# HKUST-Aerial-Robotics/A-LOAM

Hardware: AMD Instinct MI355X
Metric: HDL-64 scans/sec (whole node) (higher is better)
Workload: dtype f32 features / f64 solve

## Files before the change

a-loam_amd/binding.py:

```python
from __future__ import annotations

import ctypes as C
import os
import re
import subprocess

import numpy as np

_HERE = os.path.dirname(os.path.abspath(__file__))
_ROOT = os.path.dirname(_HERE)
LIB_PATH = os.path.join(_HERE, "lib", "libaloam_mi355x.so")
HEADER_PATH = os.path.join(_ROOT, "include", "aloam_mi355x.h")

CLOUD_FULL, CLOUD_SHARP, CLOUD_LESS_SHARP, CLOUD_FLAT, CLOUD_LESS_FLAT, CLOUD_CORNER_LAST, CLOUD_SURF_LAST = range(7)
E_ARG, E_SCAN_LINES, E_EMPTY, E_CAPACITY, E_HIP, E_STATE = -1, -2, -3, -4, -5, -6
MAP_REGISTERED, MAP_CORNER_STACK, MAP_SURF_STACK, MAP_SURROUND, MAP_FULL = 2, 3, 4, 5, 6
EXPORT_MAP, EXPORT_MAX_IDS = 16, 12
STAGE_REGISTRATION, STAGE_ODOMETRY, STAGE_MAPPING, STAGE_ALL = 1, 2, 4, 7
SEQ_RECORD_MAGIC, SEQ_RECORD_VERSION = 0x51534C41, 1
SEQ_PART_ODOMETRY, SEQ_PART_MAP = 1, 2
MAP_INFO_KEYS = ("cenW", "cenH", "cenD", "frame_count", "from_map_corner", "from_map_surf", "corner_stack", "surf_stack",
                 "corner_num0", "corner_num1", "surf_num0", "surf_num1", "lm_iterations0", "lm_iterations1", "termination0", "compactions")


# ... 316 lines not shown
        L.aloam_atlas_attach.argtypes = [vp, vp]
        L.aloam_atlas_info.argtypes = [vp, vp]
        L.aloam_places_enable.argtypes = [vp, C.c_int, C.c_float, C.c_float]
        L.aloam_places_add.argtypes = [vp, vp, C.c_int]
        L.aloam_places_match.argtypes = [vp, vp, C.c_int, vp, C.c_int, vp]
        L.aloam_places_export.argtypes = [vp, C.c_int, C.c_int, vp]
        L.aloam_places_load.argtypes = [vp, vp, C.c_int]
        L.aloam_places_clear.argtypes = [vp]
        L.aloam_places_info.argtypes = [vp, vp]
        L.aloam_save_sequences.argtypes = [vp, vp, C.c_int, vp, C.c_longlong, vp]
        L.aloam_load_sequences.argtypes = [vp, vp, C.c_int, vp, vp]
        L.aloam_get_ring_ranges.argtypes = [vp, C.c_int, vp, vp]
        L.aloam_get_curvature.argtypes = [vp, C.c_int, vp, C.c_int]
        L.aloam_get_labels.argtypes = [vp, C.c_int, vp, C.c_int]
        L.aloam_get_last_cloud_order.argtypes = [vp, C.c_int, vp]
        L.aloam_get_correspondences.argtypes = [vp, C.c_int, vp, C.c_int, ip, vp, vp, C.c_int, ip, vp]
        L.aloam_mapping_enable.argtypes = [vp, C.c_float, C.c_float, C.c_int]
        L.aloam_mapping_step.argtypes = [vp]
        L.aloam_mapping_set_pool_limit.argtypes = [vp, C.c_int]
        L.aloam_get_map_pool_info.argtypes = [vp, vp]
        L.aloam_set_map.argtypes = [vp, C.c_int, C.c_int, vp, vp, C.c_int, vp]
        L.aloam_set_map_frame.argtypes = [vp, C.c_int, vp, vp, vp, C.c_int]
        L.aloam_set_full_cloud.argtypes = [vp, C.c_int, vp, C.c_int]
        L.aloam_get_map_pose.argtypes = [vp, C.c_int, vp, vp, vp, vp]
        L.aloam_get_map_info.argtypes = [vp, C.c_int, vp]
        L.aloam_map_cube_counts.argtypes = [vp, C.c_int, C.c_int, vp]
        L.aloam_get_map_cube.argtypes = [vp, C.c_int, C.c_int, C.c_int, vp, C.c_int]
        L.aloam_get_map_cloud.argtypes = [vp, C.c_int, C.c_int, vp, C.c_int]
        L.aloam_export_poses.argtypes = [vp, vp]
        L.aloam_export_clouds.argtypes = [vp, vp, C.c_int, vp, C.c_longlong, vp]
# ... 662 lines not shown
    def pose(self, seq=0):
        qw, tw, ql, tl = np.zeros(4), np.zeros(3), np.zeros(4), np.zeros(3)
        self._check(lib().aloam_get_pose(self.h, seq, _p(qw), _p(tw), _p(ql), _p(tl)))
        return {"q_w": qw, "t_w": tw, "q_lc": ql, "t_lc": tl}

    def odom_stats(self, seq=0):
        st = AloamOdomStats()
        self._check(lib().aloam_get_odom_stats(self.h, seq, C.byref(st)))
        return {k: list(getattr(st, k)) for k, _ in AloamOdomStats._fields_}

    def last_cloud_order(self, seq=0):
        v = np.zeros(2, np.int32)
        self._check(lib().aloam_get_last_cloud_order(self.h, seq, _p(v)))
        return int(v[0]), int(v[1])

    def correspondences(self, seq=0):
        cap_e, cap_p = self.n_scans * 12, self.n_scans * 24
        e = np.zeros((cap_e, 9), np.float32); p = np.zeros((cap_p, 12), np.float32)
        eq = np.zeros(cap_e, np.int32); pq = np.zeros(cap_p, np.int32)
        ne, npl = C.c_int(0), C.c_int(0)
        self._check(lib().aloam_get_correspondences(self.h, seq, _p(e), cap_e, C.byref(ne), _p(eq), _p(p), cap_p, C.byref(npl), _p(pq)))
        return e[:ne.value].copy(), p[:npl.value].copy(), eq[:ne.value].copy(), pq[:npl.value].copy()

    def mapping_enable(self, line_res=0.4, plane_res=0.8, pool_points=262144, pool_limit=None):
        if pool_limit is not None:
            self._check(lib().aloam_mapping_set_pool_limit(self.h, int(pool_limit)))
        self._check(lib().aloam_mapping_enable(self.h, float(line_res), float(plane_res), int(pool_points)))

    def map_pool_info(self):
        v = np.zeros(4, np.int32)
# ... 101 lines not shown
```

a-loam_amd/csrc/aloam_capi.hip:

```cpp
#include <algorithm>
#include <cstdio>
#include <cstdlib>
#include <cstring>

#include "capi_internal.hpp"
#include "information_device.hpp"

namespace aloam {

hipEvent_t prof_event(aloam_ctx* c) {
  if (!c->prof_free.empty()) { hipEvent_t e = c->prof_free.back(); c->prof_free.pop_back(); return e; }
  Event e;
  (void)hipEventCreate(&e.h);
  c->prof_events.push_back(std::move(e));
  return c->prof_events.back();
}

int stage_ints(aloam_ctx* c, const int* src, int n, int* dst) {
  int* slot = nullptr;
  int ns = 0;
  if (const int rc = c->nin.acquire(c, &slot, &ns)) return rc;
  std::memcpy(slot, src, sizeof(int) * n);
  return c->nin.queue(c, ns, slot, sizeof(int) * n, dst, c->stream);
}
// ... 77 lines not shown
  int ndev = 0;
  if (hipGetDeviceCount(&ndev) != hipSuccess || ndev <= 0) { c->err = "no HIP device available (this library has no CPU fallback)"; return ALOAM_E_HIP; }
  if (cfg->device < 0 || cfg->device >= ndev) { c->err = "device ordinal out of range"; return ALOAM_E_ARG; }
  DeviceScope device_scope(c);
  HIP_TRY(c, hipStreamCreateWithFlags(&c->stream.h, hipStreamNonBlocking));
  HIP_TRY(c, hipStreamCreateWithFlags(&c->copy_stream.h, hipStreamNonBlocking));
  for (int k = 0; k < 2; ++k) {
    HIP_TRY(c, hipEventCreateWithFlags(&c->in_copied[k].h, hipEventDisableTiming));
    HIP_TRY(c, hipEventCreateWithFlags(&c->in_consumed[k].h, hipEventDisableTiming));
  }
  c->B = cfg->batch; c->max_points = cfg->max_points; c->R = cfg->n_scans;
  c->seq.assign(c->B, SeqHost{});
  c->cap = cfg->max_points + (((cfg->max_points / 32 + 15) & ~15) + 16);
  { const char* e = std::getenv("ALOAM_GRAPH_MAX_BATCH"); c->use_graph = c->B <= (e ? std::atoi(e) : 0); }
  { const char* e = std::getenv("ALOAM_GRID_OVERLAP"); c->grid_overlap = !(e && e[0] == '0') && !c->use_graph && !c->debug_sync; }
  c->NB = (c->cap + kBlockPts - 1) / kBlockPts;
  c->npad = cfg->max_ring_points <= 2059 ? 2048 : 4096;
  const size_t B = c->B, cap = c->cap, R = c->R, NB = c->NB;
  int rc = 0;
  if (const char* what = c->nin.create(sizeof(int) * B)) { c->err = std::string("input counts, ") + what; return ALOAM_E_HIP; }
  const bool reg = stages & ALOAM_STAGE_REGISTRATION, odo = stages & ALOAM_STAGE_ODOMETRY, map = stages & ALOAM_STAGE_MAPPING;
  c->grid_H[0] = R > 64 ? 8192 : 4096;
  c->grid_H[1] = c->max_points > 160000 ? 32768 : 16384;
  if ((rc = dmalloc(c, c->d_nin, B))) return rc;
  if ((rc = dmalloc(c, c->d_meta, B))) return rc;
  if ((rc = dmalloc(c, c->d_state, B))) return rc;
  if ((rc = dmalloc(c, c->d_cloud, B * cap))) return rc;
  if ((rc = dmalloc(c, c->d_exp_cnt, B * ALOAM_EXPORT_MAX_IDS))) return rc;
  if ((rc = dmalloc(c, c->d_exp_chunk, B * ALOAM_EXPORT_MAX_IDS + 1))) return rc;
  if ((rc = dmalloc(c, c->d_exp_off, B * ALOAM_EXPORT_MAX_IDS + 1))) return rc;
// ... 28 lines not shown
      if ((rc = dmalloc(c, c->d_grid_sorted3c[p][k], B * per))) return rc;
      if ((rc = dmalloc(c, c->d_grid_start3c[p][k], B * (c->grid_H[k] + 1)))) return rc;
      if ((rc = dmalloc(c, c->d_grid_flags[p][k], B * 4))) return rc;
      if ((rc = dmalloc(c, c->d_grid_walk[p][k], B * 2 * (R + 8)))) return rc;
    }
    if (c->grid_overlap) {
      HIP_TRY(c, hipStreamCreateWithFlags(&c->grid_stream.h, hipStreamNonBlocking));
      HIP_TRY(c, hipEventCreateWithFlags(&c->grid_fork.h, hipEventDisableTiming));
      HIP_TRY(c, hipEventCreateWithFlags(&c->grids_done.h, hipEventDisableTiming));
    }
    if ((rc = dmalloc(c, c->d_edges, B * R * kSharpPerRing))) return rc;
    if ((rc = dmalloc(c, c->d_planes, B * R * kFlatPerRing))) return rc;
    if ((rc = dmalloc(c, c->d_sel_sharp, B * R * kSharpPerRing))) return rc;
    if ((rc = dmalloc(c, c->d_sel_flat, B * R * kFlatPerRing))) return rc;
    if ((rc = prepare_build_grids(c->grid_H[1]))) { c->err = "k_build_grids: dynamic LDS size rejected"; return ALOAM_E_HIP; }
  }
  std::vector<OdomState> init(B);
  std::memset(init.data(), 0, sizeof(OdomState) * B);
  for (size_t b = 0; b < B; ++b) { init[b].para_q[3] = 1.0; init[b].q_w[3] = 1.0; }
  HIP_TRY(c, hipMemcpyAsync(c->d_state.get(), init.data(), sizeof(OdomState) * B, hipMemcpyHostToDevice, c->stream));
  HIP_TRY(c, hipStreamSynchronize(c->stream));
  return ALOAM_OK;
}

void aloam_destroy(aloam_ctx* c) {
  DeviceScope device_scope(c);
  if (!c) return;
  if (c->stream) (void)hipStreamSynchronize(c->stream);
  if (c->copy_stream) (void)hipStreamSynchronize(c->copy_stream);
  if (c->grid_stream) (void)hipStreamSynchronize(c->grid_stream);
// ... 184 lines not shown
```

a-loam_amd/csrc/aloam_device.hpp:

```cpp
#pragma once
#include <hip/hip_runtime.h>
#include <stdint.h>
#include "aloam_atan.hpp"

namespace aloam {

constexpr int kFrontSlots = 128 + 8;
constexpr int kBlockPts = 1024;
constexpr int kMaxRings = 128;
constexpr int kSectors = 6;
constexpr int kSharpPerSector = 2;
constexpr int kLessSharpPerSector = 20;
constexpr int kFlatPerSector = 4;
constexpr int kSharpPerRing = kSectors * kSharpPerSector;
constexpr int kLessSharpPerRing = kSectors * kLessSharpPerSector;
constexpr int kFlatPerRing = kSectors * kFlatPerSector;
constexpr int kNnTile = 1024;

enum ErrBits { kErrEmpty = 1, kErrRingCap = 2, kErrPointCap = 4, kErrInternal = 8 };

struct alignas(16) SeqMeta {
  int n_in;
  int first_kept, last_kept;
  int half_idx;
// ... 75 lines not shown
  int* grid_start3[2][2];
  int* grid_start2[2][2];
  float4* grid_sorted3c[2][2];
  int* grid_start3c[2][2];
  int* grid_flags[2][2];
  int* grid_walk[2][2];
  int grid_H_corner, grid_H_surf;
  float4* sel_sharp;
  float4* sel_flat;
  EdgeRec* edges;
  PlaneRec* planes;
  int outer;
  int last_outer;
  int lm_max_iterations;
  int distortion;
};

template <typename T>
__device__ __forceinline__ T* row_of(T* const (&buf)[2], int k, int b, long long per) { return (k ? buf[1] : buf[0]) + b * per; }
__device__ __forceinline__ const float4* corner_last(const OdomArgs& a, int b, int parity) { return row_of(a.less_sharp, parity ^ 1, b, (long long)a.R * kLessSharpPerRing); }
__device__ __forceinline__ const float4* surf_last(const OdomArgs& a, int b, int parity) { return row_of(a.less_flat, parity ^ 1, b, (long long)a.cap); }

struct GridView {
  int H;
  float4 *sorted3, *sorted2, *sorted3c;
  int *start3, *start2, *start3c, *flags, *walk;
};
template <typename T>
__device__ __forceinline__ T* grid_ptr(T* const (&buf)[2][2], int set, int which) {
  return set ? (which ? buf[1][1] : buf[1][0]) : (which ? buf[0][1] : buf[0][0]);
// ... 259 lines not shown
```

a-loam_amd/csrc/capi_internal.hpp:

```cpp
#pragma once
#include <hip/hip_runtime.h>

#include <cstdio>
#include <memory>
#include <functional>
#include <string>
#include <utility>
#include <vector>

#include "../../include/aloam_mi355x.h"
#include "aloam_device.hpp"
#include "atlas_kernels.hpp"
#include "checkpoint_kernels.hpp"
#include "export_kernels.hpp"
#include "graphapply_kernels.hpp"
#include "graphmap_kernels.hpp"
#include "graphmarginal_kernels.hpp"
#include "graphrecord_kernels.hpp"
#include "loopreg_kernels.hpp"
#include "loopsearch_kernels.hpp"
#include "mapping_kernels.hpp"
#include "odometry_kernels.hpp"
#include "places_kernels.hpp"
#include "posegraph_kernels.hpp"
// ... 191 lines not shown
  bool dense_valid = true;
  DevBuf<int> d_ringstart;
  DevBuf<float4> d_cloud; DevBuf<float> d_curv; DevBuf<int8_t> d_label;
  DevBuf<unsigned long long> d_lookback; unsigned reg_epoch = 0;
  DevBuf<int> d_ring_ticket;
  bool debug_arrays = false;
  DevBuf<float4> d_sharp, d_flat;
  DevBuf<float4> d_less_sharp[2], d_less_flat[2];
  DevBuf<OdomState> d_state;
  DevBuf<float4> d_grid_sorted3[2][2], d_grid_sorted2[2][2];
  DevBuf<int> d_grid_start3[2][2], d_grid_start2[2][2];
  DevBuf<float4> d_grid_sorted3c[2][2];
  DevBuf<int> d_grid_start3c[2][2];
  DevBuf<int> d_grid_flags[2][2], d_grid_walk[2][2];
  int grid_H[2] = {4096, 16384};
  bool grid_overlap = false;
  DevBuf<EdgeRec> d_edges; DevBuf<PlaneRec> d_planes;
  DevBuf<float4> d_sel_sharp, d_sel_flat;
  bool map_on = false;
  long long map_err_reported = 0;
  float map_line_res = 0.4f, map_plane_res = 0.8f;
  int map_levels = 0, map_stack_tile_bound = 0, map_nsegs_max = 0;
  MapPool map;
  int map_pool_limit = 1 << 26;
  int map_growths = 0;
  long long map_steps = 0;
  int nin_max = 0;
  int inject_max = 0;
  PinnedBuf<volatile int> h_map_report;
  int* d_map_report_host = nullptr;
// ... 225 lines not shown
```

a-loam_amd/csrc/capi_odometry.hip:

```cpp
#include <algorithm>
#include <cstring>
#include <functional>

#include "capi_internal.hpp"

namespace {

RegArgs reg_args(aloam_ctx* c, const void* d_scans, long long seq_stride, int pt_stride) {
  RegArgs a{};
  a.in = (const char*)d_scans; a.seq_stride = seq_stride; a.pt_stride = pt_stride;
  a.B = c->B; a.cap = c->cap; a.R = c->R; a.NB = c->NB;
  a.ring_from_field = c->cfg.ring_from_field; a.min_range = c->cfg.min_range;
  a.meta = c->d_meta.get(); a.slabs = c->d_slabs.get(); a.slab = c->slab; a.front_lb = c->d_front_lb.get(); a.front_ticket = c->d_front_ticket.get();
  a.ringstart = c->d_ringstart.get(); a.cloud = c->d_cloud.get(); a.curv = c->d_curv.get(); a.label = c->d_label.get();
  a.lookback = c->d_lookback.get(); a.epoch = c->reg_epoch; a.store_debug = c->debug_arrays ? 1 : 0; a.ring_ticket = c->d_ring_ticket.get();
  a.sharp = c->d_sharp.get(); a.flat = c->d_flat.get();
  for (int k = 0; k < 2; ++k) { a.less_sharp[k] = c->d_less_sharp[k].get(); a.less_flat[k] = c->d_less_flat[k].get(); }
  a.active = c->reg_mask;
  return a;
}

}

namespace aloam {
// ... 3 lines not shown
  a.B = c->B; a.cap = c->cap; a.R = c->R;
  a.meta = c->d_meta.get(); a.state = c->d_state.get();
  a.sharp = c->d_sharp.get(); a.flat = c->d_flat.get();
  for (int k = 0; k < 2; ++k) { a.less_sharp[k] = c->d_less_sharp[k].get(); a.less_flat[k] = c->d_less_flat[k].get(); }
  for (int p = 0; p < 2; ++p) for (int k = 0; k < 2; ++k) {
    a.grid_sorted3[p][k] = c->d_grid_sorted3[p][k].get(); a.grid_sorted2[p][k] = c->d_grid_sorted2[p][k].get(); a.grid_start3[p][k] = c->d_grid_start3[p][k].get();
    a.grid_sorted3c[p][k] = c->d_grid_sorted3c[p][k].get(); a.grid_start3c[p][k] = c->d_grid_start3c[p][k].get();
    a.grid_start2[p][k] = c->d_grid_start2[p][k].get();
    a.grid_flags[p][k] = c->d_grid_flags[p][k].get(); a.grid_walk[p][k] = c->d_grid_walk[p][k].get();
  }
  a.grid_H_corner = c->grid_H[0]; a.grid_H_surf = c->grid_H[1];
  a.edges = c->d_edges.get(); a.planes = c->d_planes.get();
  a.sel_sharp = c->d_sel_sharp.get(); a.sel_flat = c->d_sel_flat.get();
  a.lm_max_iterations = c->cfg.lm_max_iterations;
  a.distortion = c->cfg.distortion != 0;
  return a;
}

}

namespace {

int check_batch(aloam_ctx* c, const int* n_in, int stride_bytes) {
  if (const int rc = require_stage(c, ALOAM_STAGE_REGISTRATION)) return rc;
  if (stride_bytes < 12 || (stride_bytes & 3)) { c->err = "stride_bytes must be 12 (x, y, z only) or >= 16, and a multiple of 4"; return ALOAM_E_ARG; }
  if (stride_bytes == 12 && c->cfg.ring_from_field) { c->err = "ring_from_field needs the 4th float of every record: stride_bytes >= 16"; return ALOAM_E_ARG; }
  for (int b = 0; b < c->B; ++b) {
    if (n_in[b] < 0) { c->err = "negative point count"; return ALOAM_E_ARG; }
    if (n_in[b] > c->max_points) { c->err = "scan exceeds max_points"; return ALOAM_E_CAPACITY; }
  }
// ... 450 lines not shown
int aloam_get_labels(aloam_ctx* c, int seq, int* out, int cap) {
  DeviceScope device_scope(c);
  int rc = check_seq(c, seq);
  if (rc) return rc;
  if ((rc = require_stage(c, ALOAM_STAGE_REGISTRATION))) return rc;
  if (!c->debug_arrays) { c->err = "labels are only kept by aloam_scan_register*; the throughput entries (aloam_process_*) skip them"; return ALOAM_E_STATE; }
  SeqMeta m;
  if ((rc = read_seq(c, c->d_meta.get() + seq, &m))) return rc;
  const int k = m.n_cloud < cap ? m.n_cloud : cap;
  std::vector<int8_t> tmp(k > 0 ? k : 1);
  if (k > 0) HIP_TRY(c, hipMemcpy(tmp.data(), c->d_label.get() + (size_t)seq * c->cap, k, hipMemcpyDeviceToHost));
  for (int i = 0; i < k; ++i) out[i] = tmp[i];
  return m.n_cloud;
}

int aloam_get_last_cloud_order(aloam_ctx* c, int seq, int out[2]) {
  DeviceScope device_scope(c);
  int rc = check_seq(c, seq);
  if (rc) return rc;
  if (!c->d_grid_flags[0][0]) { c->err = "this context has no odometry stage"; return ALOAM_E_STATE; }
  HIP_TRY(c, hipStreamSynchronize(c->stream));
  const int set = c->seq[seq].parity;
  for (int k = 0; k < 2; ++k) {
    int f[4];
    HIP_TRY(c, hipMemcpy(f, c->d_grid_flags[set][k].get() + (size_t)seq * 4, sizeof(f), hipMemcpyDeviceToHost));
    out[k] = f[0] ? -1 : f[1];
  }
  return ALOAM_OK;
}

// ... 37 lines not shown
```

a-loam_amd/csrc/information_kernels.hip:

```cpp
#include "information_device.hpp"
#include "mapping_solve_device.hpp"
#include "odometry_kernels.hpp"
#include "odometry_solve_device.hpp"

namespace aloam {

template <bool DISTORT>
__global__ __launch_bounds__(kSolveThreads) void k_pose_information_odom(OdomArgs a, const int* __restrict__ list, aloam_pose_information* __restrict__ dst) {
  __shared__ double s_red[kSolveWaves * 28];
  const int code = list[blockIdx.x], b = code & kInfoSeqMask;
  const bool solved = (code & kInfoSolvedBit) != 0;
  double acc[28];
  for (int k = 0; k < 28; ++k) acc[k] = 0.0;
  int ne = 0, np = 0;
  if (solved) {
    const OdomState& st = a.state[b];
    double q[4] = {st.para_q[0], st.para_q[1], st.para_q[2], st.para_q[3]}, t[3] = {st.para_t[0], st.para_t[1], st.para_t[2]};
    if (DISTORT) {
#pragma unroll
      for (int k = 0; k < 4; ++k) asm volatile("" : "+v"(q[k]));
#pragma unroll
      for (int k = 0; k < 3; ++k) asm volatile("" : "+v"(t[k]));
    }
    evaluate<true, DISTORT>(a, b, q, t, acc, &ne, &np);
  }
  double cnt[2] = {(double)ne, (double)np};
  block_sum<28, kSolveWaves>(acc, s_red);
  block_sum<2, kSolveWaves>(cnt, s_red);
  if (threadIdx.x == 0) write_pose_information(dst + blockIdx.x, solved, acc, (int)cnt[0], (int)cnt[1], -1);
}

__global__ __launch_bounds__(kMapSolveThreads) void k_pose_information_map(MapArgs a, const int* __restrict__ list, aloam_pose_information* __restrict__ dst) {
  __shared__ double s_red[(kMapSolveThreads / 64) * 28];
  extern __shared__ int s_pref[];
  const int code = list[blockIdx.x], b = code & kInfoSeqMask, tid = threadIdx.x;
  const bool solved = (code & kInfoSolvedBit) != 0;
  const MapSeq& ms = a.seq[b];
  double acc[28];
  for (int k = 0; k < 28; ++k) acc[k] = 0.0;
// ... 34 lines not shown
```

a-loam_amd/csrc/odometry_kernels.hip:

```cpp
#include "aloam_device.hpp"
#include "aloam_trig.hpp"
#include "lm_device.hpp"
#include "odometry_solve_device.hpp"
#include "odometry_kernels.hpp"

namespace aloam {

#define ALOAM_PHASE(name) asm volatile("; ##PHASE " name)
#ifdef ALOAM_PHASE_CLOCK
__device__ unsigned long long g_phase_clock_odo[2][32];
#define ALOAM_BG_CLOCK(slot) do { if (threadIdx.x == 0 && blockIdx.x == 1) { atomicAdd(&g_phase_clock_odo[0][slot], (unsigned long long)__builtin_readcyclecounter()); atomicAdd(&g_phase_clock_odo[1][slot], 1ull); } } while (0)
#else
#define ALOAM_BG_CLOCK(slot) do { } while (0)
#endif
#ifdef ALOAM_ASSOC_STATS
__device__ unsigned long long g_assoc_stats[2][32];
#define ALOAM_STAT(cls, i, v) do { if ((threadIdx.x & 63) == 0) atomicAdd(&g_assoc_stats[cls][i], (unsigned long long)(v)); } while (0)
#else
#define ALOAM_STAT(cls, i, v) do { } while (0)
#endif

__device__ __forceinline__ float4 transform_to_start(const float4& p, const OdomState& st) {
  double q[4] = {st.para_q[0], st.para_q[1], st.para_q[2], st.para_q[3]};
  if (q[3] < 0.0) { q[0] = -q[0]; q[1] = -q[1]; q[2] = -q[2]; q[3] = -q[3]; }
// ... 1074 lines not shown
  const int nt = PLANE ? m.n_surf_last : m.n_corner_last;
  if (!(g.flags[0] != 0 || g.flags[1] == 2 || nt <= 0)) return;
  const int nq = PLANE ? m.n_flat : m.n_sharp;
  for (int qi = wave; qi < nq; qi += 4) associate_one<PLANE, WIDE>(a, b, qi, m, g, lane, rows[wave]);
}

template <bool DISTORT>
__global__ __launch_bounds__(kSolveThreads) void k_solve(OdomArgs a) {
  const int b = blockIdx.x, tid = threadIdx.x;
  __shared__ double s_red[kSolveWaves * 28];
  if (seq_idle(a.active, b, kSeqSolve)) return;
  OdomState& st = a.state[b];
  double q[4] = {st.para_q[0], st.para_q[1], st.para_q[2], st.para_q[3]};
  double t[3] = {st.para_t[0], st.para_t[1], st.para_t[2]};

  const LmResult lm = lm_solve_block<kSolveWaves>([&](bool with_jac, const double* qq, const double* tt, double* acc, int* ne, int* np) {
    if (with_jac) evaluate<true, DISTORT>(a, b, qq, tt, acc, ne, np); else evaluate<false, DISTORT>(a, b, qq, tt, acc, ne, np);
  }, q, t, a.lm_max_iterations, s_red);
  const int n_edges = lm.n_a, n_planes = lm.n_b, iterations = lm.iterations, successful = lm.successful, termination = lm.termination;
  const double initial_cost = lm.initial_cost, cost = lm.final_cost;

  if (tid == 0) {
    if (termination == 5) {
      for (int k = 0; k < 4; ++k) q[k] = st.para_q[k];
      for (int k = 0; k < 3; ++k) t[k] = st.para_t[k];
    }
    for (int k = 0; k < 4; ++k) st.para_q[k] = q[k];
    for (int k = 0; k < 3; ++k) st.para_t[k] = t[k];
    const int o = a.outer < 2 ? a.outer : 1;
    st.corner_corr[o] = n_edges;
    st.plane_corr[o] = n_planes;
    st.lm_iterations[o] = iterations;
// ... 65 lines not shown
}
void launch_associate(const OdomArgs& a, bool plane, hipStream_t s) {
  const int by = (a.B + 7) / 8 * 8;
  const int qcap = plane ? a.R * kFlatPerRing : a.R * kSharpPerRing;
  const bool wide = a.R > 64;
  const dim3 grid((unsigned)(qcap / 2 * by)), block(64), gridf((unsigned)a.B), blockf(256);
  const dim3 gridn((unsigned)((qcap / 2 + kPairsPerWave - 1) / kPairsPerWave), (unsigned)a.B);
  if (wide) {
    if (plane) { hipLaunchKernelGGL((k_associate_pair<true, true>), grid, block, 0, s, a); hipLaunchKernelGGL((k_associate_nearly<true, true>), gridn, block, 0, s, a); hipLaunchKernelGGL((k_associate_flagged<true, true>), gridf, blockf, 0, s, a); }
    else { hipLaunchKernelGGL((k_associate_pair<false, true>), grid, block, 0, s, a); hipLaunchKernelGGL((k_associate_nearly<false, true>), gridn, block, 0, s, a); hipLaunchKernelGGL((k_associate_flagged<false, true>), gridf, blockf, 0, s, a); }
  } else {
    if (plane) { hipLaunchKernelGGL((k_associate_pair<true, false>), grid, block, 0, s, a); hipLaunchKernelGGL((k_associate_nearly<true, false>), gridn, block, 0, s, a); hipLaunchKernelGGL((k_associate_flagged<true, false>), gridf, blockf, 0, s, a); }
    else { hipLaunchKernelGGL((k_associate_pair<false, false>), grid, block, 0, s, a); hipLaunchKernelGGL((k_associate_nearly<false, false>), gridn, block, 0, s, a); hipLaunchKernelGGL((k_associate_flagged<false, false>), gridf, blockf, 0, s, a); }
  }
}
void launch_solve(const OdomArgs& a, hipStream_t s) {
  if (a.distortion) hipLaunchKernelGGL(k_solve<true>, dim3(a.B), dim3(kSolveThreads), 0, s, a);
  else hipLaunchKernelGGL(k_solve<false>, dim3(a.B), dim3(kSolveThreads), 0, s, a);
}
}

#ifdef ALOAM_PHASE_CLOCK
extern "C" int aloam_debug_phase_clock_odo(unsigned long long* out) { return (int)hipMemcpyFromSymbol(out, HIP_SYMBOL(aloam::g_phase_clock_odo), sizeof(unsigned long long) * 64); }
#endif
#ifdef ALOAM_ASSOC_STATS
extern "C" int aloam_debug_assoc_stats(unsigned long long* out) { return (int)hipMemcpyFromSymbol(out, HIP_SYMBOL(aloam::g_assoc_stats), sizeof(unsigned long long) * 64); }
#endif
```

a-loam_amd/csrc/odometry_kernels.hpp:

```cpp
#pragma once
#include "aloam_device.hpp"

struct aloam_pose_information;

namespace aloam {
size_t build_grids_lds_bytes(int H, int R);
int prepare_build_grids(int H_surf);
enum class GridBuild { kSerialLast, kPersistentNext, kPersistentLast };
void launch_build_grids(const OdomArgs& a, GridBuild form, int wgs, hipStream_t s);
void launch_transform_queries(const OdomArgs& a, hipStream_t s);
void launch_associate(const OdomArgs& a, bool plane, hipStream_t s);
void launch_solve(const OdomArgs& a, hipStream_t s);
void launch_advance(const OdomArgs& a, hipStream_t s);
void launch_pose_information_odom(const OdomArgs& a, const int* list, int n, aloam_pose_information* dst, hipStream_t s);
void launch_set_inited(OdomState* state, int B, int inited, hipStream_t s);
}
```

a-loam_amd/csrc/odometry_solve_device.hpp:

```cpp
#pragma once
#include "aloam_device.hpp"
#include "aloam_trig.hpp"
#include "lm_device.hpp"

namespace aloam {

__device__ __forceinline__ double interpolation_ratio(float frac) { return (double)frac / 0.1; }

__device__ __forceinline__ void slerp_scales(double w, double s, double* c0, double* c1, double* dc0, double* dc1) {
  const double one = 1.0 - 2.220446049250313e-16;
  const double absD = fabs(w);
  if (absD >= one) { *c0 = 1.0 - s; *c1 = s; *dc0 = 0.0; *dc1 = 0.0; }
  else {
    const double theta = acos_port(absD), st = sin_port(theta), ct = cos_port(theta);
    const double a0 = (1.0 - s) * theta, a1 = s * theta;
    const double s0 = sin_port(a0), s1 = sin_port(a1);
    *c0 = s0 / st;
    *c1 = s1 / st;
    const double g = (w < 0.0 ? 1.0 : -1.0) / st;
    *dc0 = ((1.0 - s) * cos_port(a0) * st - s0 * ct) / (st * st) * g;
    *dc1 = (s * cos_port(a1) * st - s1 * ct) / (st * st) * g;
  }
  if (w < 0.0) { *c1 = -*c1; *dc1 = -*dc1; }
}
// ... 29 lines not shown
  }
}

__device__ __forceinline__ void deskew_jacobian_row(const double a[3], const double (*M)[4], const double q[4], double s, double J[6]) {
  double g[4];
#pragma unroll
  for (int j = 0; j < 4; ++j) g[j] = a[0] * M[0][j] + a[1] * M[1][j] + a[2] * M[2][j];
  J[0] = g[0] * q[3] - g[1] * q[2] + g[2] * q[1] - g[3] * q[0];
  J[1] = g[0] * q[2] + g[1] * q[3] - g[2] * q[0] - g[3] * q[1];
  J[2] = -g[0] * q[1] + g[1] * q[0] + g[2] * q[3] - g[3] * q[2];
  J[3] = a[0] * s; J[4] = a[1] * s; J[5] = a[2] * s;
}

constexpr int kSolveWaves = 2;
constexpr int kSolveThreads = 64 * kSolveWaves;
template <bool WITH_JAC, bool DISTORT>
__device__ void evaluate(const OdomArgs& a, int b, const double q[4], const double t[3], double* acc, int* n_edge, int* n_plane) {
  const int tid = threadIdx.x;
  const SeqMeta m = a.meta[b];
  const EdgeRec* E = a.edges + (long long)b * a.R * kSharpPerRing;
  const PlaneRec* P = a.planes + (long long)b * a.R * kFlatPerRing;
  int ne = 0, np = 0;
  for (int i = tid; i < m.n_sharp; i += kSolveThreads) {
    const EdgeRec e = E[i];
    if (!e.valid) continue;
    ++ne;
    double rcp[3], lp[3], M[3][4];
    const double s = DISTORT ? interpolation_ratio(__int_as_float(e.pad[0])) : 1.0;
    if (DISTORT) deskew_point(q, t, s, (double)e.cp[0], (double)e.cp[1], (double)e.cp[2], lp, WITH_JAC ? M : nullptr);
    else {
      quat_rotate(q, (double)e.cp[0], (double)e.cp[1], (double)e.cp[2], rcp);
      lp[0] = rcp[0] + t[0]; lp[1] = rcp[1] + t[1]; lp[2] = rcp[2] + t[2];
    }
    const double ax = e.a[0], ay = e.a[1], az = e.a[2], bx = e.b[0], by = e.b[1], bz = e.b[2];
    const double dex = ax - bx, dey = ay - by, dez = az - bz;
    const double inv = 1.0 / sqrt(dex * dex + dey * dey + dez * dez);
    const double ux = lp[0] - ax, uy = lp[1] - ay, uz = lp[2] - az, vx = lp[0] - bx, vy = lp[1] - by, vz = lp[2] - bz;
    const double r0 = (uy * vz - uz * vy) * inv, r1 = (uz * vx - ux * vz) * inv, r2 = (ux * vy - uy * vx) * inv;
    double rho0, rho1;
    huber(r0 * r0 + r1 * r1 + r2 * r2, &rho0, &rho1);
    acc[27] += 0.5 * rho0;
    if (WITH_JAC) {
      const double wx = -dex * inv, wy = -dey * inv, wz = -dez * inv;
      const double A[3][3] = {{0, -wz, wy}, {wz, 0, -wx}, {-wy, wx, 0}};
      const double Bm[3][3] = {{0, 2 * rcp[2], -2 * rcp[1]}, {-2 * rcp[2], 0, 2 * rcp[0]}, {2 * rcp[1], -2 * rcp[0], 0}};
      const double rr[3] = {r0, r1, r2};
#pragma unroll
      for (int row = 0; row < 3; ++row) {
        double J[6];
        if (DISTORT) deskew_jacobian_row(A[row], M, q, s, J);
        else {
#pragma unroll
          for (int c = 0; c < 3; ++c) {
            J[c] = A[row][0] * Bm[0][c] + A[row][1] * Bm[1][c] + A[row][2] * Bm[2][c];
            J[3 + c] = A[row][c];
          }
        }
        add_row(acc, J, rr[row], rho1);
      }
    }
  }
  for (int i = tid; i < m.n_flat; i += kSolveThreads) {
    const PlaneRec p = P[i];
    if (!p.valid) continue;
    ++np;
    const double jx = p.j[0], jy = p.j[1], jz = p.j[2];
    const double e1x = jx - (double)p.l[0], e1y = jy - (double)p.l[1], e1z = jz - (double)p.l[2];
    const double e2x = jx - (double)p.m[0], e2y = jy - (double)p.m[1], e2z = jz - (double)p.m[2];
    double nx = e1y * e2z - e1z * e2y, ny = e1z * e2x - e1x * e2z, nz = e1x * e2y - e1y * e2x;
    const double len = sqrt(nx * nx + ny * ny + nz * nz);
    nx /= len; ny /= len; nz /= len;
    double rcp[3] = {0.0, 0.0, 0.0}, lp[3], M[3][4];
    const double s = DISTORT ? interpolation_ratio(__int_as_float(p.pad[0])) : 1.0;
    if (DISTORT) deskew_point(q, t, s, (double)p.cp[0], (double)p.cp[1], (double)p.cp[2], lp, WITH_JAC ? M : nullptr);
    else {
      quat_rotate(q, (double)p.cp[0], (double)p.cp[1], (double)p.cp[2], rcp);
      lp[0] = rcp[0] + t[0]; lp[1] = rcp[1] + t[1]; lp[2] = rcp[2] + t[2];
    }
    const double r = (lp[0] - jx) * nx + (lp[1] - jy) * ny + (lp[2] - jz) * nz;
    double rho0, rho1;
    huber(r * r, &rho0, &rho1);
    acc[27] += 0.5 * rho0;
    if (WITH_JAC) {
      double J[6];
      const double nn[3] = {nx, ny, nz};
      if (DISTORT) deskew_jacobian_row(nn, M, q, s, J);
      else { J[0] = 2.0 * (nz * rcp[1] - ny * rcp[2]); J[1] = 2.0 * (nx * rcp[2] - nz * rcp[0]); J[2] = 2.0 * (ny * rcp[0] - nx * rcp[1]); J[3] = nx; J[4] = ny; J[5] = nz; }
      add_row(acc, J, r, rho1);
    }
  }
  *n_edge = ne;
  *n_plane = np;
}

}
```

include/aloam_mi355x.h:

```cpp
#ifndef ALOAM_MI355X_H_
#define ALOAM_MI355X_H_

#ifdef __cplusplus
extern "C" {
#endif

typedef struct aloam_ctx aloam_ctx;

enum {
  ALOAM_OK = 0,
  ALOAM_E_ARG = -1,
  ALOAM_E_SCAN_LINES = -2,
  ALOAM_E_EMPTY = -3,
  ALOAM_E_CAPACITY = -4,
  ALOAM_E_HIP = -5,
  ALOAM_E_STATE = -6
};

typedef struct aloam_config {
  int n_scans;
  float min_range;
  int ring_from_field;
  int batch;
  int max_points;
// ... 377 lines not shown
} aloam_graph_robust_result;
void aloam_graph_robust_default_options(aloam_graph_robust_options* opt);
int aloam_graph_optimize_robust(aloam_ctx* ctx, const int* seqs, int n, const aloam_graph_options* opt, const aloam_graph_robust_options* robust,
                                aloam_graph_robust_result* dst , double* weights_dst , long long weights_stride);

int aloam_get_ring_ranges(aloam_ctx* ctx, int seq, int* start, int* count);
int aloam_get_curvature(aloam_ctx* ctx, int seq, float* out, int cap);
int aloam_get_labels(aloam_ctx* ctx, int seq, int* out, int cap);
int aloam_get_correspondences(aloam_ctx* ctx, int seq, float* edges, int cap_edges, int* n_edges, int* edge_query,
                              float* planes, int cap_planes, int* n_planes, int* plane_query);
int aloam_get_map_factors(aloam_ctx* ctx, int seq, double* lines, int cap_lines, int* n_lines, double* planes, int cap_planes, int* n_planes);
int aloam_graph_loop_export_target(aloam_ctx* ctx, int slot, int feature_class, float* dst_xyzw, long long cap, int* count);

int aloam_get_last_cloud_order(aloam_ctx* ctx, int seq, int out[2]);

int aloam_profile_enable(aloam_ctx* ctx, int on);
int aloam_profile_kernel_count(void);
const char* aloam_profile_kernel_name(int kernel);
int aloam_profile_get(aloam_ctx* ctx, int kernel, double* total_ms, long long* launches, double* algorithmic_bytes);

#ifdef __cplusplus
}
#endif
#endif
```

Baseline: 136,300.

## Stage solve correspondences in LDS with precomputed normals and prefetched loads

The LM solve kernel now decodes edge and plane records once on the first evaluation and caches the coordinates, line inverse lengths and plane normals in dynamic LDS, up to a budget. Later iterations read from LDS instead of re-reading global records and recomputing normals. Records that do not fit are still fetched from global memory, with a software prefetch of two records ahead. Every evaluation now also computes the Jacobian. The large dynamic LDS allocation may reduce occupancy, and the deeper prefetch adds register pressure.

New measurement: 139,400 (median of 6 runs). 2.3% higher.

```diff
diff --git a/a-loam_amd/binding.py b/a-loam_amd/binding.py
--- a/a-loam_amd/binding.py
+++ b/a-loam_amd/binding.py
@@ -354,6 +354,8 @@
         L.aloam_get_curvature.argtypes = [vp, C.c_int, vp, C.c_int]
         L.aloam_get_labels.argtypes = [vp, C.c_int, vp, C.c_int]
         L.aloam_get_last_cloud_order.argtypes = [vp, C.c_int, vp]
+        if hasattr(L, "aloam_get_solve_lds"):
+            L.aloam_get_solve_lds.argtypes = [vp, vp]
         L.aloam_get_correspondences.argtypes = [vp, C.c_int, vp, C.c_int, ip, vp, vp, C.c_int, ip, vp]
         L.aloam_mapping_enable.argtypes = [vp, C.c_float, C.c_float, C.c_int]
         L.aloam_mapping_step.argtypes = [vp]
@@ -1046,6 +1048,11 @@
         self._check(lib().aloam_get_last_cloud_order(self.h, seq, _p(v)))
         return int(v[0]), int(v[1])
 
+    def solve_lds(self):
+        v = np.zeros(3, np.int32)
+        self._check(lib().aloam_get_solve_lds(self.h, _p(v)))
+        return int(v[0]), int(v[1]), int(v[2])
+
     def correspondences(self, seq=0):
         cap_e, cap_p = self.n_scans * 12, self.n_scans * 24
         e = np.zeros((cap_e, 9), np.float32); p = np.zeros((cap_p, 12), np.float32)
diff --git a/a-loam_amd/csrc/aloam_capi.hip b/a-loam_amd/csrc/aloam_capi.hip
--- a/a-loam_amd/csrc/aloam_capi.hip
+++ b/a-loam_amd/csrc/aloam_capi.hip
@@ -115,6 +115,7 @@
   c->cap = cfg->max_points + (((cfg->max_points / 32 + 15) & ~15) + 16);
   { const char* e = std::getenv("ALOAM_GRAPH_MAX_BATCH"); c->use_graph = c->B <= (e ? std::atoi(e) : 0); }
   { const char* e = std::getenv("ALOAM_GRID_OVERLAP"); c->grid_overlap = !(e && e[0] == '0') && !c->use_graph && !c->debug_sync; }
+  { const char* e = std::getenv("ALOAM_SOLVE_STAGE"); c->solve_stage = !(e && e[0] == '0'); }
   c->NB = (c->cap + kBlockPts - 1) / kBlockPts;
   c->npad = cfg->max_ring_points <= 2059 ? 2048 : 4096;
   const size_t B = c->B, cap = c->cap, R = c->R, NB = c->NB;
@@ -173,6 +174,7 @@
     if ((rc = dmalloc(c, c->d_sel_sharp, B * R * kSharpPerRing))) return rc;
     if ((rc = dmalloc(c, c->d_sel_flat, B * R * kFlatPerRing))) return rc;
     if ((rc = prepare_build_grids(c->grid_H[1]))) { c->err = "k_build_grids: dynamic LDS size rejected"; return ALOAM_E_HIP; }
+    if (c->solve_stage && (rc = prepare_solve())) { c->err = "k_solve: dynamic LDS size rejected"; return ALOAM_E_HIP; }
   }
   std::vector<OdomState> init(B);
   std::memset(init.data(), 0, sizeof(OdomState) * B);
diff --git a/a-loam_amd/csrc/aloam_device.hpp b/a-loam_amd/csrc/aloam_device.hpp
--- a/a-loam_amd/csrc/aloam_device.hpp
+++ b/a-loam_amd/csrc/aloam_device.hpp
@@ -113,6 +113,7 @@
   int last_outer;
   int lm_max_iterations;
   int distortion;
+  int solve_stage;
 };
 
 template <typename T>
diff --git a/a-loam_amd/csrc/capi_internal.hpp b/a-loam_amd/csrc/capi_internal.hpp
--- a/a-loam_amd/csrc/capi_internal.hpp
+++ b/a-loam_amd/csrc/capi_internal.hpp
@@ -229,6 +229,7 @@
   DevBuf<int> d_grid_start3c[2][2];
   DevBuf<int> d_grid_flags[2][2], d_grid_walk[2][2];
   int grid_H[2] = {4096, 16384};
+  bool solve_stage = true;
   bool grid_overlap = false;
   DevBuf<EdgeRec> d_edges; DevBuf<PlaneRec> d_planes;
   DevBuf<float4> d_sel_sharp, d_sel_flat;
diff --git a/a-loam_amd/csrc/capi_odometry.hip b/a-loam_amd/csrc/capi_odometry.hip
--- a/a-loam_amd/csrc/capi_odometry.hip
+++ b/a-loam_amd/csrc/capi_odometry.hip
@@ -41,6 +41,7 @@
   a.sel_sharp = c->d_sel_sharp.get(); a.sel_flat = c->d_sel_flat.get();
   a.lm_max_iterations = c->cfg.lm_max_iterations;
   a.distortion = c->cfg.distortion != 0;
+  a.solve_stage = c->solve_stage ? 1 : 0;
   return a;
 }
 
@@ -521,6 +522,13 @@
   return m.n_cloud;
 }
 
+int aloam_get_solve_lds(aloam_ctx* c, int out[3]) {
+  if (!c || !out) return ALOAM_E_ARG;
+  if (!c->d_edges) { c->err = "this context has no odometry stage"; return ALOAM_E_STATE; }
+  solve_launch_lds(odom_args(c), out);
+  return ALOAM_OK;
+}
+
 int aloam_get_last_cloud_order(aloam_ctx* c, int seq, int out[2]) {
   DeviceScope device_scope(c);
   int rc = check_seq(c, seq);
diff --git a/a-loam_amd/csrc/information_kernels.hip b/a-loam_amd/csrc/information_kernels.hip
--- a/a-loam_amd/csrc/information_kernels.hip
+++ b/a-loam_amd/csrc/information_kernels.hip
@@ -22,7 +22,7 @@
 #pragma unroll
       for (int k = 0; k < 3; ++k) asm volatile("" : "+v"(t[k]));
     }
-    evaluate<true, DISTORT>(a, b, q, t, acc, &ne, &np);
+    evaluate<true, DISTORT, 0, DISTORT ? 0 : 1>(a, b, q, t, acc, &ne, &np);
   }
   double cnt[2] = {(double)ne, (double)np};
   block_sum<28, kSolveWaves>(acc, s_red);
diff --git a/a-loam_amd/csrc/odometry_kernels.hip b/a-loam_amd/csrc/odometry_kernels.hip
--- a/a-loam_amd/csrc/odometry_kernels.hip
+++ b/a-loam_amd/csrc/odometry_kernels.hip
@@ -1112,8 +1112,11 @@
   double q[4] = {st.para_q[0], st.para_q[1], st.para_q[2], st.para_q[3]};
   double t[3] = {st.para_t[0], st.para_t[1], st.para_t[2]};
 
-  const LmResult lm = lm_solve_block<kSolveWaves>([&](bool with_jac, const double* qq, const double* tt, double* acc, int* ne, int* np) {
-    if (with_jac) evaluate<true, DISTORT>(a, b, qq, tt, acc, ne, np); else evaluate<false, DISTORT>(a, b, qq, tt, acc, ne, np);
+  SolveKeep keep = {a.solve_stage ? solve_stage(a.R, DISTORT) : SolveStage{0, 0, 0}, 0u, 0u};
+  bool first = true;
+  const LmResult lm = lm_solve_block<kSolveWaves>([&](bool, const double* qq, const double* tt, double* acc, int* ne, int* np) __attribute__((always_inline)) {
+    if (first) { first = false; evaluate<true, DISTORT, 1, kSolveAhead>(a, b, qq, tt, acc, ne, np, &keep); }
+    else evaluate<true, DISTORT, 2, kSolveAhead>(a, b, qq, tt, acc, ne, np, &keep);
   }, q, t, a.lm_max_iterations, s_red);
   const int n_edges = lm.n_a, n_planes = lm.n_b, iterations = lm.iterations, successful = lm.successful, termination = lm.termination;
   const double initial_cost = lm.initial_cost, cost = lm.final_cost;
@@ -1209,9 +1212,21 @@
     else { hipLaunchKernelGGL((k_associate_pair<false, false>), grid, block, 0, s, a); hipLaunchKernelGGL((k_associate_nearly<false, false>), gridn, block, 0, s, a); hipLaunchKernelGGL((k_associate_flagged<false, false>), gridf, blockf, 0, s, a); }
   }
 }
+int prepare_solve() {
+  const int most = kSolveLdsBudget - kSolveStaticLds;
+  if (hipFuncSetAttribute((const void*)k_solve<true>, hipFuncAttributeMaxDynamicSharedMemorySize, most) != hipSuccess) return -1;
+  return hipFuncSetAttribute((const void*)k_solve<false>, hipFuncAttributeMaxDynamicSharedMemorySize, most) == hipSuccess ? 0 : -1;
+}
+void solve_launch_lds(const OdomArgs& a, int out[3]) {
+  const SolveStage st = a.solve_stage ? solve_stage(a.R, a.distortion != 0) : SolveStage{0, 0, 0};
+  out[0] = st.plane_slots; out[1] = st.edge_slots; out[2] = st.bytes;
+}
 void launch_solve(const OdomArgs& a, hipStream_t s) {
-  if (a.distortion) hipLaunchKernelGGL(k_solve<true>, dim3(a.B), dim3(kSolveThreads), 0, s, a);
-  else hipLaunchKernelGGL(k_solve<false>, dim3(a.B), dim3(kSolveThreads), 0, s, a);
+  int keep[3];
+  solve_launch_lds(a, keep);
+  const size_t lds = (size_t)keep[2];
+  if (a.distortion) hipLaunchKernelGGL(k_solve<true>, dim3(a.B), dim3(kSolveThreads), lds, s, a);
+  else hipLaunchKernelGGL(k_solve<false>, dim3(a.B), dim3(kSolveThreads), lds, s, a);
 }
 }
 
diff --git a/a-loam_amd/csrc/odometry_kernels.hpp b/a-loam_amd/csrc/odometry_kernels.hpp
--- a/a-loam_amd/csrc/odometry_kernels.hpp
+++ b/a-loam_amd/csrc/odometry_kernels.hpp
@@ -10,6 +10,8 @@
 void launch_build_grids(const OdomArgs& a, GridBuild form, int wgs, hipStream_t s);
 void launch_transform_queries(const OdomArgs& a, hipStream_t s);
 void launch_associate(const OdomArgs& a, bool plane, hipStream_t s);
+int prepare_solve();
+void solve_launch_lds(const OdomArgs& a, int out[3]);
 void launch_solve(const OdomArgs& a, hipStream_t s);
 void launch_advance(const OdomArgs& a, hipStream_t s);
 void launch_pose_information_odom(const OdomArgs& a, const int* list, int n, aloam_pose_information* dst, hipStream_t s);
diff --git a/a-loam_amd/csrc/odometry_solve_device.hpp b/a-loam_amd/csrc/odometry_solve_device.hpp
--- a/a-loam_amd/csrc/odometry_solve_device.hpp
+++ b/a-loam_amd/csrc/odometry_solve_device.hpp
@@ -67,19 +67,71 @@
 
 constexpr int kSolveWaves = 2;
 constexpr int kSolveThreads = 64 * kSolveWaves;
-template <bool WITH_JAC, bool DISTORT>
-__device__ void evaluate(const OdomArgs& a, int b, const double q[4], const double t[3], double* acc, int* n_edge, int* n_plane) {
+constexpr int kSolveAhead = 2;
+
+constexpr int kSolveLdsBudget = 80 * 1024;
+constexpr int kSolveStaticLds = kSolveWaves * 28 * (int)sizeof(double);
+constexpr int kPlaneKeepBytes = 6 * 4 + 3 * 8, kEdgeKeepBytes = 9 * 4 + 8;
+struct SolveStage { int plane_slots, edge_slots, bytes; };
+__host__ __device__ constexpr int solve_slots(int records) { return (records + kSolveThreads - 1) / kSolveThreads; }
+__host__ __device__ constexpr SolveStage solve_stage(int R, bool distort) {
+  const int per_plane = (kPlaneKeepBytes + (distort ? 4 : 0)) * kSolveThreads, per_edge = (kEdgeKeepBytes + (distort ? 4 : 0)) * kSolveThreads;
+  const int room = kSolveLdsBudget - kSolveStaticLds;
+  const int all_p = solve_slots(R * kFlatPerRing), all_e = solve_slots(R * kSharpPerRing);
+  const int np = room / per_plane < all_p ? room / per_plane : all_p;
+  const int ne = (room - np * per_plane) / per_edge < all_e ? (room - np * per_plane) / per_edge : all_e;
+  return SolveStage{np, ne, np * per_plane + ne * per_edge};
+}
+static_assert(solve_slots(kMaxRings * kFlatPerRing) <= 32 && solve_slots(kMaxRings * kSharpPerRing) <= 32, "a thread's validity masks are 32 bits per class");
+struct SolveKeep { SolveStage lds; unsigned plane_valid, edge_valid; };
+
+struct EdgeFetch { float4 v[3]; };
+struct PlaneFetch { float4 v[4]; };
+struct EdgeKept { float cp[3], a[3], b[3], frac; double inv; };
+struct PlaneKept { float cp[3], j[3], frac; double n[3]; };
+
+template <int AHEAD, class Load, class Term>
+__device__ __forceinline__ void walk_ahead(int k0, int k1, Load&& load, Term&& term) {
+  if (k0 >= k1) return;
+  if constexpr (AHEAD == 0) {
+    for (int k = k0; k < k1; ++k) term(load(k), k);
+    return;
+  }
+  decltype(load(0)) r[AHEAD > 0 ? AHEAD : 1];
+#pragma unroll
+  for (int d = 0; d < AHEAD; ++d) r[d] = load(k0 + d < k1 ? k0 + d : k1 - 1);
+  for (int k = k0; k < k1; k += AHEAD) {
+#pragma unroll
+    for (int d = 0; d < AHEAD; ++d) {
+      if (k + d < k1) {
+        const auto cur = r[d];
+        r[d] = load(k + d + AHEAD < k1 ? k + d + AHEAD : k1 - 1);
+        term(cur, k + d);
+      }
+    }
+  }
+}
+
+template <bool WITH_JAC, bool DISTORT, int STAGE = 0, int AHEAD = 1>
+__device__ __forceinline__ void evaluate(const OdomArgs& a, int b, const double q[4], const double t[3], double* acc, int* n_edge, int* n_plane, SolveKeep* keep = nullptr) {
+  constexpr int T = kSolveThreads, NPF = 6 + (DISTORT ? 1 : 0), NEF = 9 + (DISTORT ? 1 : 0);
+  extern __shared__ double s_keep[];
   const int tid = threadIdx.x;
   const SeqMeta m = a.meta[b];
-  const EdgeRec* E = a.edges + (long long)b * a.R * kSharpPerRing;
-  const PlaneRec* P = a.planes + (long long)b * a.R * kFlatPerRing;
+  const float4* E = reinterpret_cast<const float4*>(a.edges + (long long)b * a.R * kSharpPerRing);
+  const float4* P = reinterpret_cast<const float4*>(a.planes + (long long)b * a.R * kFlatPerRing);
+  const int slots_e = tid < m.n_sharp ? (m.n_sharp - tid + T - 1) / T : 0, slots_p = tid < m.n_flat ? (m.n_flat - tid + T - 1) / T : 0;
+  const int kept_p = STAGE ? keep->lds.plane_slots : 0, kept_e = STAGE ? keep->lds.edge_slots : 0;
+  double* const s_pn = s_keep + tid;
+  double* const s_inv = s_keep + kept_p * 3 * T + tid;
+  float* const s_pf = reinterpret_cast<float*>(s_keep + (kept_p * 3 + kept_e) * T) + tid;
+  float* const s_ef = reinterpret_cast<float*>(s_keep + (kept_p * 3 + kept_e) * T) + kept_p * NPF * T + tid;
   int ne = 0, np = 0;
-  for (int i = tid; i < m.n_sharp; i += kSolveThreads) {
-    const EdgeRec e = E[i];
-    if (!e.valid) continue;
+
+  auto edge_term = [&](const EdgeKept& e) {
     ++ne;
     double rcp[3], lp[3], M[3][4];
-    const double s = DISTORT ? interpolation_ratio(__int_as_float(e.pad[0])) : 1.0;
+    const double s = DISTORT ? interpolation_ratio(e.frac) : 1.0;
     if (DISTORT) deskew_point(q, t, s, (double)e.cp[0], (double)e.cp[1], (double)e.cp[2], lp, WITH_JAC ? M : nullptr);
     else {
       quat_rotate(q, (double)e.cp[0], (double)e.cp[1], (double)e.cp[2], rcp);
@@ -87,7 +139,7 @@
     }
     const double ax = e.a[0], ay = e.a[1], az = e.a[2], bx = e.b[0], by = e.b[1], bz = e.b[2];
     const double dex = ax - bx, dey = ay - by, dez = az - bz;
-    const double inv = 1.0 / sqrt(dex * dex + dey * dey + dez * dez);
+    const double inv = e.inv;
     const double ux = lp[0] - ax, uy = lp[1] - ay, uz = lp[2] - az, vx = lp[0] - bx, vy = lp[1] - by, vz = lp[2] - bz;
     const double r0 = (uy * vz - uz * vy) * inv, r1 = (uz * vx - ux * vz) * inv, r2 = (ux * vy - uy * vx) * inv;
     double rho0, rho1;
@@ -112,19 +164,45 @@
         add_row(acc, J, rr[row], rho1);
       }
     }
-  }
-  for (int i = tid; i < m.n_flat; i += kSolveThreads) {
-    const PlaneRec p = P[i];
-    if (!p.valid) continue;
+  };
+  auto edge_record = [&](const EdgeFetch& f, int k) {
+    if (!__float_as_int(f.v[2].y)) return;
+    EdgeKept e = {{f.v[0].x, f.v[0].y, f.v[0].z}, {f.v[0].w, f.v[1].x, f.v[1].y}, {f.v[1].z, f.v[1].w, f.v[2].x}, f.v[2].z, 0.0};
+    const double dex = (double)e.a[0] - (double)e.b[0], dey = (double)e.a[1] - (double)e.b[1], dez = (double)e.a[2] - (double)e.b[2];
+    e.inv = 1.0 / sqrt(dex * dex + dey * dey + dez * dez);
+    if (STAGE == 1 && k < kept_e) {
+      keep->edge_valid |= 1u << k;
+      float* const f32 = s_ef + k * NEF * T;
+#pragma unroll
+      for (int c = 0; c < 3; ++c) { f32[c * T] = e.cp[c]; f32[(3 + c) * T] = e.a[c]; f32[(6 + c) * T] = e.b[c]; }
+      if (DISTORT) f32[9 * T] = e.frac;
+      s_inv[k * T] = e.inv;
+    }
+    edge_term(e);
+  };
+  auto edge_global = [&](int k) { const float4* p = E + (long long)(tid + k * T) * 3; return EdgeFetch{{p[0], p[1], p[2]}}; };
+  int first_e = 0;
+  if (STAGE == 1) keep->edge_valid = 0;
+  if (STAGE == 2) {
+    first_e = slots_e < kept_e ? slots_e : kept_e;
+    walk_ahead<1>(0, first_e, [&](int k) {
+      EdgeKept e;
+      const float* const f32 = s_ef + k * NEF * T;
+#pragma unroll
+      for (int c = 0; c < 3; ++c) { e.cp[c] = f32[c * T]; e.a[c] = f32[(3 + c) * T]; e.b[c] = f32[(6 + c) * T]; }
+      e.frac = DISTORT ? f32[9 * T] : 0.0f;
+      e.inv = s_inv[k * T];
+      return e;
+    }, [&](const EdgeKept& e, int k) { if (keep->edge_valid >> k & 1u) edge_term(e); });
+  }
+  walk_ahead<AHEAD>(first_e, slots_e, edge_global, edge_record);
+
+  auto plane_term = [&](const PlaneKept& p) {
     ++np;
     const double jx = p.j[0], jy = p.j[1], jz = p.j[2];
-    const double e1x = jx - (double)p.l[0], e1y = jy - (double)p.l[1], e1z = jz - (double)p.l[2];
-    const double e2x = jx - (double)p.m[0], e2y = jy - (double)p.m[1], e2z = jz - (double)p.m[2];
-    double nx = e1y * e2z - e1z * e2y, ny = e1z * e2x - e1x * e2z, nz = e1x * e2y - e1y * e2x;
-    const double len = sqrt(nx * nx + ny * ny + nz * nz);
-    nx /= len; ny /= len; nz /= len;
+    const double nx = p.n[0], ny = p.n[1], nz = p.n[2];
     double rcp[3] = {0.0, 0.0, 0.0}, lp[3], M[3][4];
-    const double s = DISTORT ? interpolation_ratio(__int_as_float(p.pad[0])) : 1.0;
+    const double s = DISTORT ? interpolation_ratio(p.frac) : 1.0;
     if (DISTORT) deskew_point(q, t, s, (double)p.cp[0], (double)p.cp[1], (double)p.cp[2], lp, WITH_JAC ? M : nullptr);
     else {
       quat_rotate(q, (double)p.cp[0], (double)p.cp[1], (double)p.cp[2], rcp);
@@ -141,7 +219,40 @@
       else { J[0] = 2.0 * (nz * rcp[1] - ny * rcp[2]); J[1] = 2.0 * (nx * rcp[2] - nz * rcp[0]); J[2] = 2.0 * (ny * rcp[0] - nx * rcp[1]); J[3] = nx; J[4] = ny; J[5] = nz; }
       add_row(acc, J, r, rho1);
     }
-  }
+  };
+  auto plane_record = [&](const PlaneFetch& f, int k) {
+    if (!__float_as_int(f.v[3].x)) return;
+    PlaneKept p = {{f.v[0].x, f.v[0].y, f.v[0].z}, {f.v[0].w, f.v[1].x, f.v[1].y}, f.v[3].y, {0.0, 0.0, 0.0}};
+    const double jx = p.j[0], jy = p.j[1], jz = p.j[2];
+    const double e1x = jx - (double)f.v[1].z, e1y = jy - (double)f.v[1].w, e1z = jz - (double)f.v[2].x;
+    const double e2x = jx - (double)f.v[2].y, e2y = jy - (double)f.v[2].z, e2z = jz - (double)f.v[2].w;
+    double nx = e1y * e2z - e1z * e2y, ny = e1z * e2x - e1x * e2z, nz = e1x * e2y - e1y * e2x;
+    const double len = sqrt(nx * nx + ny * ny + nz * nz);
+    p.n[0] = nx / len; p.n[1] = ny / len; p.n[2] = nz / len;
+    if (STAGE == 1 && k < kept_p) {
+      keep->plane_valid |= 1u << k;
+      float* const f32 = s_pf + k * NPF * T;
+#pragma unroll
+      for (int c = 0; c < 3; ++c) { f32[c * T] = p.cp[c]; f32[(3 + c) * T] = p.j[c]; s_pn[(k * 3 + c) * T] = p.n[c]; }
+      if (DISTORT) f32[6 * T] = p.frac;
+    }
+    plane_term(p);
+  };
+  auto plane_global = [&](int k) { const float4* p = P + (long long)(tid + k * T) * 4; return PlaneFetch{{p[0], p[1], p[2], p[3]}}; };
+  int first_p = 0;
+  if (STAGE == 1) keep->plane_valid = 0;
+  if (STAGE == 2) {
+    first_p = slots_p < kept_p ? slots_p : kept_p;
+    walk_ahead<1>(0, first_p, [&](int k) {
+      PlaneKept p;
+      const float* const f32 = s_pf + k * NPF * T;
+#pragma unroll
+      for (int c = 0; c < 3; ++c) { p.cp[c] = f32[c * T]; p.j[c] = f32[(3 + c) * T]; p.n[c] = s_pn[(k * 3 + c) * T]; }
+      p.frac = DISTORT ? f32[6 * T] : 0.0f;
+      return p;
+    }, [&](const PlaneKept& p, int k) { if (keep->plane_valid >> k & 1u) plane_term(p); });
+  }
+  walk_ahead<AHEAD>(first_p, slots_p, plane_global, plane_record);
   *n_edge = ne;
   *n_plane = np;
 }
diff --git a/include/aloam_mi355x.h b/include/aloam_mi355x.h
--- a/include/aloam_mi355x.h
+++ b/include/aloam_mi355x.h
@@ -415,6 +415,8 @@
 
 int aloam_get_last_cloud_order(aloam_ctx* ctx, int seq, int out[2]);
 
+int aloam_get_solve_lds(aloam_ctx* ctx, int out[3]);
+
 int aloam_profile_enable(aloam_ctx* ctx, int on);
 int aloam_profile_kernel_count(void);
 const char* aloam_profile_kernel_name(int kernel);
```
